# Etienne-bdt/Simple-VAE-RS

Hardware: NVIDIA B200
Metric: train patches/sec (64x64 SR CondVAE, device-timed) (higher is better)
Workload: dtype bf16

## Files before the change

### include/svrs_b200.h

```cpp
#ifndef SVRS_B200_H
#define SVRS_B200_H

#include <stdint.h>

#ifdef __cplusplus
extern "C" {
#endif

#define SVRS_F32 0
#define SVRS_BF16 1

#define SVRS_ACT_NONE 0
#define SVRS_ACT_SIGMOID 1
#define SVRS_ACT_HARDTANH7 2

#define SVRS_E_ARG (-1)
#define SVRS_E_CUDA (-2)
#define SVRS_E_UNSUPPORTED (-3)

const char* svrs_last_error(void);
int svrs_abi_version(void);
int64_t svrs_launch_count(void);
void svrs_trace_reset(int enable);
const char* svrs_trace(void);
int svrs_device_cc(int dev);

int svrs_nchw_to_nhwc(const void* src, int src_dtype, int64_t src_ld, void* dst, int dst_dtype,
                      int N, int C, int H, int W, void* stream);
int svrs_nhwc_to_nchw(const void* src, int src_dtype, void* dst, int dst_dtype, int64_t dst_ld,
                      int N, int C, int H, int W, int accumulate, void* stream);

int svrs_pack_weights(const float* w, int d0, int d1, int kk, void* p01, void* p10, int dtype,
                      void* stream);

int svrs_pack_job_bytes(void);
int svrs_pack_weights_multi(const void* jobs, int njobs, int total_tiles, int max_kk, int dtype, void* stream);
int svrs_unpack_grads_multi(const void* jobs, int njobs, int total_tiles, int max_kk, void* stream);

void svrs_set_tc_enabled(int enabled);
void svrs_set_halo_mode(int mode);
int svrs_tc_would_run(int dtype, int K, int Nc, int OH, int OW);

int svrs_conv2d_fprop(const void* x, const void* w_kn, const void* w_nk, const float* bias, void* y, int dtype,
                      int N, int H, int W, int Cin, int Cout, int ksize, int act, void* stream);
int svrs_conv2d_fprop_ex(const void* x, const void* w_kn, const void* w_nk, const float* bias, void* y, int dtype,
                         int out_dtype, float* y_nchw, int64_t y_nchw_ld, double* bn_sums,
                         int N, int H, int W, int Cin, int Cout, int ksize, int act, void* stream);
int svrs_conv2d_dgrad(const void* dy, const void* w_kn, const void* w_nk, void* dx, int dtype,
                      int N, int H, int W, int Cin, int Cout, int ksize, void* stream);
int svrs_conv2d_wgrad(const void* x, const void* dy, float* dw, float* dw_packed, float* db, int dtype,
                      int N, int H, int W, int Cin, int Cout, int ksize, int ksplit, void* stream);


int svrs_convT2d_fprop(const void* x, const void* w_kn, const void* w_nk, const float* bias, void* y, int dtype,
                       int N, int H, int W, int Cin, int Cout, int act, void* stream);
int svrs_convT2d_fprop_ex(const void* x, const void* w_kn, const void* w_nk, const float* bias, void* y, int dtype,
                          double* bn_sums, int N, int H, int W, int Cin, int Cout, int act, void* stream);
int svrs_convT2d_dgrad(const void* dy, const void* w_kn, const void* w_nk, void* dx, int dtype,
                       int N, int H, int W, int Cin, int Cout, void* stream);
int svrs_convT2d_wgrad(const void* x, const void* dy, float* dw, float* dw_packed, float* db, int dtype,
                       int N, int H, int W, int Cin, int Cout, int ksplit, void* stream);

int svrs_conv2d_wgrad_layout(int dtype, int N, int H, int W, int Cin, int Cout, int ksize);
int svrs_convT2d_wgrad_layout(int dtype, int N, int H, int W, int Cin, int Cout);

#define SVRS_BN_REPLICAS 8
int svrs_bn_stats(const void* x, int dtype, int64_t M, int C, double* sums, void* stream);
int svrs_bn_finalize_train(const double* sums, int64_t M, int C, const float* gamma, const float* beta,
                           float eps, float momentum, float* running_mean, float* running_var,
                           int64_t* num_batches_tracked, int n_updates,
                           float* scale, float* shift, float* mean, float* invstd, void* stream);
int svrs_bn_apply_train(const void* x, void* y, int dtype, int64_t M, int64_t M_stat, int C, const double* sums,
                        const float* gamma, const float* beta, float eps, float momentum,
                        float* running_mean, float* running_var, int64_t* num_batches_tracked, int n_updates,
                        int relu, float* scale, float* shift, float* mean, float* invstd, void* stream);
int svrs_bn_finalize_eval(int C, const float* gamma, const float* beta, float eps,
                          const float* running_mean, const float* running_var,
                          float* scale, float* shift, void* stream);
int svrs_bn_apply(const void* x, void* y, int dtype, int64_t M, int C, const float* scale,
                  const float* shift, int relu, void* stream);
int svrs_bn_bwd_reduce(const void* x, const void* dy, int dtype, int64_t M, int C, const float* scale,
                       const float* shift, const float* mean, const float* invstd, int relu,
                       double* sums, void* stream);
int svrs_bn_bwd_apply(const void* x, const void* dy, void* dx, int dtype, int64_t M, int64_t M_stat, int C,
                      const float* scale, const float* shift, const float* mean, const float* invstd,
                      const float* gamma, int relu, const double* sums, float* dgamma, float* dbeta,
                      void* stream);

int svrs_reparam_fwd(const float* enc, const float* eps, float* z, int64_t z_ld, float* eps_out, int B, int Wd,
                     uint64_t seed, uint32_t stream_id, uint64_t sample_offset, const int64_t* step_ptr,
                     void* stream);
int svrs_reparam_bwd(const float* enc, const float* eps, const float* dz, int64_t dz_ld, float* denc, int B, int Wd,
                     uint64_t seed, uint32_t stream_id, uint64_t sample_offset, const int64_t* step_ptr,
                     void* stream);
int svrs_philox_normal(float* out, int B, int Wd, uint64_t seed, uint32_t stream_id,
                       uint64_t sample_offset, const int64_t* step_ptr, void* stream);

int svrs_elbo_fwd(const void* recon_x, const void* x, int dt_x, int dt_tx, int64_t n_x,
                  const void* recon_y, const void* y, int dt_y, int dt_ty, int64_t n_y,
                  const float* mu1, const float* lv1, int64_t ld1, int W1,
                  const float* mu2, const float* lv2, int64_t ld2,
                  const float* mu3, const float* lv3, int64_t ld3, int W2,
                  int B, double* acc, void* stream);
int svrs_elbo_finalize(const double* acc, int64_t n_x, int64_t n_y, int B, const float* gammas ,
                       float* out5, void* stream);
int svrs_elbo_bwd(const void* recon_x, const void* x, int dt_x, int dt_tx, int64_t n_x, void* d_recon_x, int dt_dx,
                  const void* recon_y, const void* y, int dt_y, int dt_ty, int64_t n_y, void* d_recon_y, int dt_dy,
                  const float* mu1, const float* lv1, int64_t ld1, int W1, float* d_mu1, float* d_lv1, int64_t dld1,
                  const float* mu2, const float* lv2, int64_t ld2, float* d_mu2, float* d_lv2, int64_t dld2,
                  const float* mu3, const float* lv3, int64_t ld3, int W2, float* d_mu3, float* d_lv3, int64_t dld3,
                  int B, const double* acc, const float* gammas, const float* gout, float* d_gammas,
                  int act, void* stream);

int svrs_sumsq(const float* g, int64_t n, double* acc , void* stream);
int svrs_clip_adam(float* p, const float* g, float* m, float* v, int64_t n, const double* sumsq,
                   float max_norm, float grad_scale, float lr, float beta1, float beta2, float eps,
                   const int64_t* step_ptr, void* stream);
int svrs_step_increment(int64_t* step_ptr, void* stream);
int svrs_step_begin(int64_t* step_ptr, double* norm_acc, void* stream);
int svrs_adam_job_bytes(void);
int svrs_adam_tile_rows(void);
int svrs_adam_tile_cols(int kk);
int svrs_adam_multi(const void* jobs, int njobs, int total_tiles, int max_kk, float* p, const float* g, float* m, float* v,
                    int pack_dtype, const double* sumsq, float max_norm, float grad_scale, float lr, float beta1,
                    float beta2, float eps, const int64_t* step_ptr, void* stream);

int svrs_grid_patch_normalize(const void* tiles, int src_is_i16, void* dst, int dst_dtype, int nhwc,
                              int T, int C, int S, int P, void* stream);

int svrs_patch_gather_normalize(const void* tiles, int src_is_i16, int T, int C, int S, int P,
                                const int32_t* origins, int npatch, float* out_nchw_f32, float* out_nhwc_f32,
                                void* out_nhwc_bf16, void* stream);

int svrs_sample_latents(const float* mu3, const float* lv3, int64_t ld3, const float* yflat, int64_t ldy,
                        const float* eps, float* stack, int B, int S, int Wz, uint64_t seed, int stream_id,
                        uint64_t sample_offset, const int64_t* step_ptr, void* stream);
int svrs_sample_tail_splits(int B, int S, int H, int W);
int64_t svrs_sample_tail_scratch_floats(int B, int H, int W, int splits);
int svrs_sample_tail_stats(const void* x, int dtype, const void* w_kn, const float* bias, const float* target_nhwc,
                           int B, int S, int H, int W, int Cin, int Cout, int splits, float* scratch,
                           float* mean_nchw, float* std_map, float* mae_map, float* mse_map, float* bias_map,
                           float* sample0_nchw, void* stream);

int64_t svrs_ssim_workspace_doubles(int N, int C, int H, int W, int win);
int svrs_ssim(const float* a, const float* b, int N, int C, int H, int W, int win, float data_range, double* workspace,
              double* out, void* stream);

int svrs_act_bwd(const void* y, const void* dy, void* dx, int dtype, int act, int64_t n, void* stream);

int svrs_copy2d(const void* src, int src_dtype, int64_t src_ld, void* dst, int dst_dtype, int64_t dst_ld,
                int64_t rows, int cols, int accumulate, void* stream);

int svrs_fill_zero(void* p, int64_t bytes, void* stream);
int svrs_axpy_f32(float* y, const float* x, float a, int64_t n, void* stream);
int svrs_cast(const void* src, int src_dtype, void* dst, int dst_dtype, int64_t n, void* stream);

int svrs_debug_tap_geometry(int form, int N, int H, int W, int Cr, int Cw, int64_t* out, int cap);

#ifdef __cplusplus
}
#endif
#endif
```

### simple-vae-rs_b200/svrs_native/csrc/conv_simt.cu

```cuda
#include "common.cuh"
#include <stdlib.h>
#include "taps.cuh"
#include "tc_ptx.cuh"

namespace svrs {

struct ConvArgs {
    const void* in;
    void* out;
    const void* w;
    const float* bias;
    int act;
    double* bn_sums;
    TapGeom g;
};

constexpr int BK = 16;

}
#include "conv_narrow.cuh"
namespace svrs {
extern int g_tc_enabled_narrow;

template <typename T, int BM, int BN>
// ... 594 lines not shown
#pragma unroll
    for (int j = 0; j < TPW; ++j)
#pragma unroll
        for (int ia = 0; ia < CA; ++ia)
#pragma unroll
            for (int ib = 0; ib < CB; ++ib) {
                float v = acc[j][ia][ib];
#pragma unroll
                for (int o = 16; o > 0; o >>= 1) v += __shfl_xor_sync(0xffffffffu, v, o);
                if (lane == 0) red[warp][(j * CA + ia) * CB + ib] = v;
            }
    __syncwarp();
    for (int e = lane; e < TPW * CA * CB; e += 32) {
        const int ib = e % CB, ia = (e / CB) % CA, j = e / (CA * CB);
        if (t0 + j < pb.ntaps) atomicAdd(&a.dw[((long long)ia * CB + ib) * a.KK + t0 + j], red[warp][e]);
    }
}

template <typename T>
static bool try_launch_wgrad_narrow(const WgradArgs& a, cudaStream_t st, int& rc) {
    const TapGeom& g = a.g;
    const int Ca = g.Nc, Cb = g.K, ntaps = g.prob[0].ntaps;
    const long long ohw = (long long)g.OH * g.OW;
    static const bool disabled = getenv("SVRS_NO_NARROW") != nullptr;
    if (disabled) return false;
    if (g.nprob != 1 || ohw % 32 != 0 || (long long)g.N * ohw >= (1ll << 31) || ntaps > 16) return false;
    const int groups = (int)((long long)g.N * ohw / 32);
    const int warps = (Ca == 4 && Cb == 4) ? (ntaps + 3) / 4 : ntaps;
    const int wpc = warps % 3 == 0 ? 3 : (warps >= 4 ? 4 : warps);
    const int zg = (warps + wpc - 1) / wpc;
    int per_sm = 65536 / (128 * 32 * wpc);
    if (per_sm > 5) per_sm = 5;
    int gx = (num_sms() * per_sm + zg - 1) / zg;
    if (gx > groups) gx = groups;
    dim3 grid(gx, 1, zg);
    if (Ca == 4 && Cb == 16) SVRS_LAUNCH((wgrad_narrow_kernel<T, 4, 16, 1>), grid, 32 * wpc, 0, st, a);
    else if (Ca == 16 && Cb == 4) SVRS_LAUNCH((wgrad_narrow_kernel<T, 16, 4, 1>), grid, 32 * wpc, 0, st, a);
    else if (Ca == 4 && Cb == 4) SVRS_LAUNCH((wgrad_narrow_kernel<T, 4, 4, 4>), grid, 32 * wpc, 0, st, a);
    else return false;
    rc = check_launch("wgrad_narrow_kernel");
    return true;
}

template <typename T>
static int launch_wgrad_direct(const WgradArgs& a, cudaStream_t st) {
    const TapGeom& g = a.g;
    const long long M = (long long)g.N * g.OH * g.OW;
    const int subs = ((g.Nc + 3) / 4) * ((g.K + 3) / 4);
    const int ntaps = g.prob[0].ntaps;
    int SUB = subs <= 1 ? 1 : subs <= 4 ? 4 : subs <= 16 ? 16 : 64;
    int groups = (subs + SUB - 1) / SUB;
    const int L = 256 / SUB;
    long long want = 8LL * num_sms();
    long long split = (want + (long long)ntaps * groups - 1) / ((long long)ntaps * groups);
    long long maxsplit = (M + 8LL * L - 1) / (8LL * L);
    if (split > maxsplit) split = maxsplit;
    if (split < 1) split = 1;
    if (split > 65535) split = 65535;
    dim3 grid(ntaps, (unsigned)split, groups);
    if (SUB == 1) SVRS_LAUNCH((wgrad_direct_kernel<T, 1>), grid, 256, 0, st, a);
    else if (SUB == 4) SVRS_LAUNCH((wgrad_direct_kernel<T, 4>), grid, 256, 0, st, a);
    else if (SUB == 16) SVRS_LAUNCH((wgrad_direct_kernel<T, 16>), grid, 256, 0, st, a);
    else SVRS_LAUNCH((wgrad_direct_kernel<T, 64>), grid, 256, 0, st, a);
    return check_launch("wgrad_direct_kernel");
}

static int launch_wgrad(WgradArgs& a, int dtype, int ksplit, cudaStream_t st) {
    const TapGeom& g = a.g;
    long long M = (long long)g.N * g.OH * g.OW;
    if (M == 0) return 0;
    if ((g.Nc <= 16 || g.K <= 16) && ksplit <= 0) {
        a.ksplit = 1;
        int rc = 0;
        if (dtype == SVRS_F32 ? try_launch_wgrad_narrow<float>(a, st, rc) : try_launch_wgrad_narrow<__nv_bfloat16>(a, st, rc)) return rc;
        return dtype == SVRS_F32 ? launch_wgrad_direct<float>(a, st) : launch_wgrad_direct<__nv_bfloat16>(a, st);
    }
    int tiles = ((g.Nc + 63) / 64) * ((g.K + 63) / 64);
    int ntaps = g.prob[0].ntaps;
    if (ksplit <= 0) {
        long long want = 4LL * num_sms();
        long long base = (long long)tiles * ntaps;
        ksplit = (int)((want + base - 1) / base);
        long long maxsplit = (M + 255) / 256;
        if (ksplit > maxsplit) ksplit = (int)maxsplit;
        if (ksplit < 1) ksplit = 1;
    }
    a.ksplit = ksplit;
    dim3 grid(tiles, ntaps, ksplit);
    if (dtype == SVRS_F32) SVRS_LAUNCH((wgrad_taps_kernel<float>), grid, 256, 0, st, a);
    else SVRS_LAUNCH((wgrad_taps_kernel<__nv_bfloat16>), grid, 256, 0, st, a);
    return check_launch("wgrad_taps_kernel");
}

template <typename T>
__global__ void __launch_bounds__(256) colsum_vec_kernel(const T* __restrict__ x, long long M, int C,
                                                          float* __restrict__ out, long long rows_per_block) {
    pdl_entry();
    __shared__ float red[256][4];
    const int cg = C / 4;
    const int q = threadIdx.x % cg, lane = threadIdx.x / cg, lanes = 256 / cg;
    const long long r0 = (long long)blockIdx.x * rows_per_block;
    long long r1 = r0 + rows_per_block;
    if (r1 > M) r1 = M;
    float4 s = make_float4(0.f, 0.f, 0.f, 0.f);
    for (long long r = r0 + lane; r < r1; r += lanes) {
        float4 v = ld4(x + r * C + q * 4);
        s.x += v.x; s.y += v.y; s.z += v.z; s.w += v.w;
    }
    red[threadIdx.x][0] = s.x; red[threadIdx.x][1] = s.y; red[threadIdx.x][2] = s.z; red[threadIdx.x][3] = s.w;
    __syncthreads();
    if (lane == 0) {
        for (int l = 1; l < lanes; ++l) {
            s.x += red[l * cg + q][0]; s.y += red[l * cg + q][1]; s.z += red[l * cg + q][2]; s.w += red[l * cg + q][3];
        }
        atomicAdd(&out[q * 4 + 0], s.x); atomicAdd(&out[q * 4 + 1], s.y);
        atomicAdd(&out[q * 4 + 2], s.z); atomicAdd(&out[q * 4 + 3], s.w);
    }
}

static int launch_colsum(const void* x, int dtype, long long M, int C, float* out, cudaStream_t st) {
    if (M == 0 || C == 0) return 0;
    if (C % 4 == 0 && C / 4 <= 256 && 256 % (C / 4) == 0) {
        int lanes = 256 / (C / 4);
        long long blocks = (M + (long long)lanes * 16 - 1) / ((long long)lanes * 16);
        long long cap = 4LL * num_sms();
        if (blocks > cap) blocks = cap;
        if (blocks < 1) blocks = 1;
        long long rpb = (M + blocks - 1) / blocks;
        blocks = (M + rpb - 1) / rpb;
        if (dtype == SVRS_F32) SVRS_LAUNCH((colsum_vec_kernel<float>), (unsigned)blocks, 256, 0, st, (const float*)x, M, C, out, rpb);
        else SVRS_LAUNCH((colsum_vec_kernel<__nv_bfloat16>), (unsigned)blocks, 256, 0, st, (const __nv_bfloat16*)x, M, C, out, rpb);
        return check_launch("colsum_vec_kernel");
    }
    long long blocks = (M + 511) / 512;
    long long cap = 8LL * num_sms();
    if (blocks > cap) blocks = cap;
    long long rpb = (M + blocks - 1) / blocks;
    blocks = (M + rpb - 1) / rpb;
    if (dtype == SVRS_F32) SVRS_LAUNCH((colsum_kernel<float>), (unsigned)blocks, 256, 0, st, (const float*)x, M, C, out, rpb);
    else SVRS_LAUNCH((colsum_kernel<__nv_bfloat16>), (unsigned)blocks, 256, 0, st, (const __nv_bfloat16*)x, M, C, out, rpb);
    return check_launch("colsum_kernel");
}

}

namespace svrs {
bool tc_supported(int dtype, int K, int Nc, int OW, int OH);
int launch_conv_tc(int form, const void* in, const void* w_nk, const float* bias, void* out, int N, int H, int W, int Cr, int Cw,
                   int act, const ConvExtra& ex, cudaStream_t st);
bool wgrad_tc_supported(int dtype, int Ca, int Cb, int OW, int OH);
int launch_wgrad_tc(const TapGeom& g, const void* gmat, const void* x, float* dw, int packed, int KK, float* db, cudaStream_t st);
bool wgrad_halo_supported(const TapGeom& g, int KK);
int launch_wgrad3_halo(const TapGeom& g, const void* gmat, const void* x, float* dw, int packed, float* db, cudaStream_t st);
static int g_tc_enabled = 1;
int g_tc_enabled_narrow = 1;
static inline bool use_tc(const void* w_nk, int dtype, int K, int Nc, int OW, int OH) {
    return g_tc_enabled && w_nk != nullptr && !((K == 4 || Nc == 4) && K <= 16 && Nc <= 16) && tc_supported(dtype, K, Nc, OW, OH);
}
}

using namespace svrs;

static bool dtype_ok(int d) { return d == SVRS_F32 || d == SVRS_BF16; }

namespace svrs { void set_halo_mode(int m); }
extern "C" void svrs_set_tc_enabled(int enabled) { svrs::g_tc_enabled = enabled; svrs::g_tc_enabled_narrow = enabled; }
extern "C" void svrs_set_halo_mode(int mode) { svrs::set_halo_mode(mode); }
extern "C" int svrs_tc_would_run(int dtype, int K, int Nc, int OH, int OW) {
    return svrs::g_tc_enabled && svrs::tc_supported(dtype, K, Nc, OW, OH) ? 1 : 0;
}

extern "C" int svrs_conv2d_fprop_ex(const void* x, const void* w_kn, const void* w_nk, const float* bias, void* y, int dtype,
                                    int out_dtype, float* y_nchw, int64_t y_nchw_ld, double* bn_sums,
                                    int N, int H, int W, int Cin, int Cout, int ksize, int act, void* stream) {
    SVRS_CHECK_ARG(x && w_kn && (y || y_nchw) && dtype_ok(dtype) && dtype_ok(out_dtype), "conv2d_fprop: null pointer or bad dtype");
    SVRS_CHECK_ARG(ksize == 3 || (ksize == 4 && H % 2 == 0 && W % 2 == 0), "conv2d_fprop: ksize must be 3, or 4 with even H,W");
    SVRS_CHECK_ARG(N >= 0 && H > 0 && W > 0 && Cin > 0 && Cout > 0, "conv2d_fprop: bad dims");
    if (N > 0 && use_tc(w_nk, dtype, Cin, Cout, ksize == 3 ? W : W / 2, ksize == 3 ? H : H / 2)) {
        if (out_dtype != dtype) { set_error("conv2d_fprop_ex: the tensor-core kernels store bf16 (use y_nchw for an fp32 copy)"); return SVRS_E_UNSUPPORTED; }
        ConvExtra ex;
        ex.out2 = y_nchw; ex.out2_ld = y_nchw_ld; ex.bn_sums = bn_sums;
        return launch_conv_tc(ksize == 3 ? 0 : 2, x, w_nk, bias, y, N, H, W, Cin, Cout, act, ex, (cudaStream_t)stream);
    }
    if (y_nchw || !y) { set_error("conv2d_fprop_ex: the NCHW second output needs the tensor-core kernel (Cin=%d Cout=%d)", Cin, Cout); return SVRS_E_UNSUPPORTED; }
    ConvArgs a;
    a.in = x; a.out = y; a.w = w_kn; a.bias = bias; a.act = act; a.bn_sums = bn_sums;
    if (ksize == 3) geom_conv3(a.g, N, H, W, Cin, Cout, false);
    else geom_conv4s2(a.g, N, H, W, Cin, Cout);
    return launch_conv(a, dtype, (cudaStream_t)stream, out_dtype);
}

extern "C" int svrs_conv2d_fprop(const void* x, const void* w_kn, const void* w_nk, const float* bias, void* y, int dtype,
                                 int N, int H, int W, int Cin, int Cout, int ksize, int act, void* stream) {
    return svrs_conv2d_fprop_ex(x, w_kn, w_nk, bias, y, dtype, dtype, nullptr, 0, nullptr, N, H, W, Cin, Cout, ksize, act, stream);
}

extern "C" int svrs_conv2d_dgrad(const void* dy, const void* w_kn, const void* w_nk, void* dx, int dtype,
                                 int N, int H, int W, int Cin, int Cout, int ksize, void* stream) {
    SVRS_CHECK_ARG(dy && w_kn && dx && dtype_ok(dtype), "conv2d_dgrad: null pointer or bad dtype");
    SVRS_CHECK_ARG(ksize == 3 || (ksize == 4 && H % 2 == 0 && W % 2 == 0), "conv2d_dgrad: ksize must be 3, or 4 with even H,W");
    if (N > 0 && ksize == 3 && use_tc(w_nk, dtype, Cout, Cin, W, H))
        return launch_conv_tc(1, dy, w_nk, nullptr, dx, N, H, W, Cout, Cin, SVRS_ACT_NONE, ConvExtra(), (cudaStream_t)stream);
    if (N > 0 && ksize == 4 && use_tc(w_nk, dtype, Cout, Cin, W / 2, H / 2))
        return launch_conv_tc(3, dy, w_nk, nullptr, dx, N, H / 2, W / 2, Cout, Cin, SVRS_ACT_NONE, ConvExtra(), (cudaStream_t)stream);
    ConvArgs a;
    a.in = dy; a.out = dx; a.w = w_kn; a.bias = nullptr; a.act = SVRS_ACT_NONE; a.bn_sums = nullptr;
    if (ksize == 3) geom_conv3(a.g, N, H, W, Cout, Cin, true);
    else geom_convT4s2(a.g, N, H / 2, W / 2, Cout, Cin);
    return launch_conv(a, dtype, (cudaStream_t)stream);
}

extern "C" int svrs_convT2d_fprop_ex(const void* x, const void* w_kn, const void* w_nk, const float* bias, void* y, int dtype,
                                     double* bn_sums, int N, int H, int W, int Cin, int Cout, int act, void* stream) {
    SVRS_CHECK_ARG(x && w_kn && y && dtype_ok(dtype), "convT2d_fprop: null pointer or bad dtype");
    if (N > 0 && use_tc(w_nk, dtype, Cin, Cout, W, H)) {
        ConvExtra ex;
        ex.bn_sums = bn_sums;
        return launch_conv_tc(3, x, w_nk, bias, y, N, H, W, Cin, Cout, act, ex, (cudaStream_t)stream);
    }
    ConvArgs a;
    a.in = x; a.out = y; a.w = w_kn; a.bias = bias; a.act = act; a.bn_sums = bn_sums;
    geom_convT4s2(a.g, N, H, W, Cin, Cout);
    return launch_conv(a, dtype, (cudaStream_t)stream);
}

extern "C" int svrs_convT2d_fprop(const void* x, const void* w_kn, const void* w_nk, const float* bias, void* y, int dtype,
                                  int N, int H, int W, int Cin, int Cout, int act, void* stream) {
    return svrs_convT2d_fprop_ex(x, w_kn, w_nk, bias, y, dtype, nullptr, N, H, W, Cin, Cout, act, stream);
}

extern "C" int svrs_convT2d_dgrad(const void* dy, const void* w_kn, const void* w_nk, void* dx, int dtype,
                                  int N, int H, int W, int Cin, int Cout, void* stream) {
    SVRS_CHECK_ARG(dy && w_kn && dx && dtype_ok(dtype), "convT2d_dgrad: null pointer or bad dtype");
    if (N > 0 && use_tc(w_nk, dtype, Cout, Cin, W, H))
        return launch_conv_tc(2, dy, w_nk, nullptr, dx, N, 2 * H, 2 * W, Cout, Cin, SVRS_ACT_NONE, ConvExtra(), (cudaStream_t)stream);
    ConvArgs a;
    a.in = dy; a.out = dx; a.w = w_kn; a.bias = nullptr; a.act = SVRS_ACT_NONE; a.bn_sums = nullptr;
    geom_conv4s2(a.g, N, 2 * H, 2 * W, Cout, Cin);
    return launch_conv(a, dtype, (cudaStream_t)stream);
}

extern "C" int svrs_conv2d_wgrad(const void* x, const void* dy, float* dw, float* dw_packed, float* db, int dtype,
                                 int N, int H, int W, int Cin, int Cout, int ksize, int ksplit, void* stream) {
    SVRS_CHECK_ARG(x && dy && dtype_ok(dtype), "conv2d_wgrad: null pointer or bad dtype");
    SVRS_CHECK_ARG(ksize == 3 || (ksize == 4 && H % 2 == 0 && W % 2 == 0), "conv2d_wgrad: bad ksize");
    int rc = 0;
    if (dw) {
        WgradArgs a;
        a.gmat = dy; a.x = x; a.dw = dw; a.KK = ksize * ksize;
        if (ksize == 3) geom_conv3(a.g, N, H, W, Cin, Cout, false);
        else geom_conv4s2(a.g, N, H, W, Cin, Cout);
        const bool fold_db = db != nullptr && Cout % 8 == 0;
        if (g_tc_enabled_narrow && ksplit <= 0 && wgrad16_takes(dtype, N, H, W, Cin, Cout, ksize)) {
            rc = launch_wgrad16(x, dy, dw, db, N, H, W, Cin, (cudaStream_t)stream);
            db = nullptr;
        } else if (g_tc_enabled && N > 0 && dtype == SVRS_BF16 && wgrad_halo_supported(a.g, a.KK)) {
            rc = launch_wgrad3_halo(a.g, dy, x, dw_packed ? dw_packed : dw, dw_packed != nullptr, fold_db ? db : nullptr, (cudaStream_t)stream);
            if (fold_db) db = nullptr;
        } else if (g_tc_enabled && N > 0 && wgrad_tc_supported(dtype, Cout, Cin, a.g.OW, a.g.OH)) {
            rc = launch_wgrad_tc(a.g, dy, x, dw_packed ? dw_packed : dw, dw_packed != nullptr, a.KK, fold_db ? db : nullptr, (cudaStream_t)stream);
            if (fold_db) db = nullptr;
        } else if (g_tc_enabled_narrow && N > 0 && ksplit <= 0 && wgrad_narrow_mma_takes(a.g, dtype)) {
            rc = launch_wgrad_narrow_mma(a, db, (cudaStream_t)stream);
            db = nullptr;
        } else
            rc = launch_wgrad(a, dtype, ksplit, (cudaStream_t)stream);
        if (rc) return rc;
    }
    if (db) {
        int s = ksize == 3 ? 1 : 2;
        rc = launch_colsum(dy, dtype, (long long)N * (H / s) * (W / s), Cout, db, (cudaStream_t)stream);
    }
    return rc;
}

extern "C" int svrs_convT2d_wgrad(const void* x, const void* dy, float* dw, float* dw_packed, float* db, int dtype,
                                  int N, int H, int W, int Cin, int Cout, int ksplit, void* stream) {
    SVRS_CHECK_ARG(x && dy && dtype_ok(dtype), "convT2d_wgrad: null pointer or bad dtype");
    int rc = 0;
    if (dw) {
        WgradArgs a;
        a.gmat = x; a.x = dy; a.dw = dw; a.KK = 16;
        geom_conv4s2(a.g, N, 2 * H, 2 * W, Cout, Cin);
        if (g_tc_enabled && N > 0 && wgrad_tc_supported(dtype, Cin, Cout, a.g.OW, a.g.OH))
            rc = launch_wgrad_tc(a.g, x, dy, dw_packed ? dw_packed : dw, dw_packed != nullptr, 16, nullptr, (cudaStream_t)stream);
        else
            rc = launch_wgrad(a, dtype, ksplit, (cudaStream_t)stream);
        if (rc) return rc;
    }
    if (db) rc = launch_colsum(dy, dtype, (long long)N * 4 * H * W, Cout, db, (cudaStream_t)stream);
    return rc;
}

extern "C" int svrs_conv2d_wgrad_layout(int dtype, int N, int H, int W, int Cin, int Cout, int ksize) {
    if (!(ksize == 3 || (ksize == 4 && H % 2 == 0 && W % 2 == 0)) || N <= 0) return 0;
    if (g_tc_enabled_narrow && wgrad16_takes(dtype, N, H, W, Cin, Cout, ksize)) return 0;
    TapGeom g;
    if (ksize == 3) geom_conv3(g, N, H, W, Cin, Cout, false);
    else geom_conv4s2(g, N, H, W, Cin, Cout);
    if (g_tc_enabled && dtype == SVRS_BF16 && wgrad_halo_supported(g, ksize * ksize)) return 1;
    if (g_tc_enabled && wgrad_tc_supported(dtype, Cout, Cin, g.OW, g.OH)) return 1;
    return 0;
}
extern "C" int svrs_convT2d_wgrad_layout(int dtype, int N, int H, int W, int Cin, int Cout) {
    if (N <= 0) return 0;
    TapGeom g;
    geom_conv4s2(g, N, 2 * H, 2 * W, Cout, Cin);
    return (g_tc_enabled && wgrad_tc_supported(dtype, Cin, Cout, g.OW, g.OH)) ? 1 : 0;
}

extern "C" int svrs_debug_tap_geometry(int form, int N, int H, int W, int Cr, int Cw, int64_t* out, int cap) {
    SVRS_CHECK_ARG(out && form >= 0 && form <= 3, "debug_tap_geometry: bad args");
    TapGeom g;
    if (form == 0) geom_conv3(g, N, H, W, Cr, Cw, false);
    else if (form == 1) geom_conv3(g, N, H, W, Cr, Cw, true);
    else if (form == 2) geom_conv4s2(g, N, H, W, Cr, Cw);
    else geom_convT4s2(g, N, H, W, Cr, Cw);
    int n = 0;
    auto put = [&](long long v) { if (n < cap) out[n] = v; ++n; };
    put(g.N); put(g.OH); put(g.OW); put(g.IH); put(g.IW); put(g.K); put(g.Nc); put(g.nprob);
    put(g.o_sn); put(g.o_sy); put(g.o_sx); put(g.i_sn); put(g.i_sy); put(g.i_sx);
    for (int p = 0; p < g.nprob; ++p) {
        put(g.prob[p].out_off); put(g.prob[p].ntaps);
        for (int t = 0; t < g.prob[p].ntaps; ++t) {
            put(g.prob[p].taps[t].in_off); put(g.prob[p].taps[t].w_off); put(g.prob[p].taps[t].dy); put(g.prob[p].taps[t].dx);
        }
    }
    SVRS_CHECK_ARG(n <= cap, "debug_tap_geometry: buffer too small (%d needed)", n);
    return n;
}
```

### simple-vae-rs_b200/svrs_native/lib.py

```python
from __future__ import annotations

import ctypes
import os
import re
from typing import Dict, List, Tuple

HERE = os.path.dirname(os.path.abspath(__file__))
ROOT = os.path.dirname(os.path.dirname(HERE))
HEADER = os.path.join(ROOT, "include", "svrs_b200.h")
LIB_PATH = os.path.join(HERE, "libsvrs_b200.so")

F32, BF16 = 0, 1
ACT_NONE, ACT_SIGMOID, ACT_HARDTANH7 = 0, 1, 2

_SCALARS = {
    "int": ctypes.c_int,
    "int64_t": ctypes.c_int64,
    "uint64_t": ctypes.c_uint64,
    "uint32_t": ctypes.c_uint32,
    "float": ctypes.c_float,
}


class SvrsError(RuntimeError):
    pass


class SvrsUnsupported(SvrsError):
    """SVRS_E_UNSUPPORTED (-3): the kernel that takes this shape cannot provide a requested optional extra; nothing was
    enqueued.  Callers use the separate kernels instead (never a CPU path)."""


def parse_header(path: str = HEADER) -> Dict[str, Tuple[str, List[Tuple[str, str]]]]:
    src = open(path).read()
    src = re.sub(r"/\*.*?\*/", " ", src, flags=re.S)
    src = re.sub(r"//[^\n]*", " ", src)
    protos = {}
    for m in re.finditer(r"(const\s+char\s*\*|int64_t|int|void)\s+(svrs_\w+)\s*\(([^;{]*?)\)\s*;", src, flags=re.S):
        ret, name, args = m.group(1), m.group(2), m.group(3)
        arglist = []
        args = " ".join(args.split())
        if args and args != "void":
            for a in args.split(","):
                a = a.strip()
                mm = re.match(r"(.*?)(\w+)$", a)
                ty, an = mm.group(1).strip(), mm.group(2)
                arglist.append((ty.replace(" *", "*"), an))
        protos[name] = ("char*" if "char" in ret else ret.strip(), arglist)
    return protos


def _ctype(ty: str):
    if "*" in ty:
        return ctypes.c_void_p
    ty = ty.replace("const", "").strip()
    return _SCALARS[ty]


class _Lib:
    def __init__(self):
        self._dll = None
        self.protos = parse_header()
        self.timing = None
        self.timing_pad_cycles = 0

    def load(self):
        if self._dll is not None:
            return self._dll
        if not os.path.exists(LIB_PATH):
            raise SvrsError(
                f"{LIB_PATH} is missing: the sm_100a kernel library has not been built "
                f"(run `python simple-vae-rs_b200/svrs_native/build.py`). There is no CPU/eager fallback.")
        dll = ctypes.CDLL(LIB_PATH)
        for name, (ret, args) in self.protos.items():
            fn = getattr(dll, name)
            fn.argtypes = [_ctype(t) for t, _ in args]
            fn.restype = {"char*": ctypes.c_char_p, "void": None, "int64_t": ctypes.c_int64}.get(ret, ctypes.c_int)
        self._dll = dll
        return dll

    def last_error(self) -> str:
        return self.load().svrs_last_error().decode()

    def __getattr__(self, name):
        full = "svrs_" + name
        if full not in self.protos:
            raise AttributeError(name)
        fn = getattr(self.load(), full)
        if self.protos[full][0] != "int" or full in ("svrs_abi_version", "svrs_device_cc", "svrs_debug_tap_geometry", "svrs_tc_would_run", "svrs_pack_job_bytes", "svrs_launch_count", "svrs_adam_job_bytes", "svrs_adam_tile_rows", "svrs_adam_tile_cols",
                                                  "svrs_conv2d_wgrad_layout", "svrs_convT2d_wgrad_layout", "svrs_sample_tail_splits"):
            setattr(self, name, fn)
            return fn

        def call(*a, _fn=fn, _n=full):
            if self.timing is not None:
                import torch
                e0, e1 = torch.cuda.Event(enable_timing=True), torch.cuda.Event(enable_timing=True)
                if self.timing_pad_cycles:
                    torch.cuda._sleep(self.timing_pad_cycles)
                dll = self.load()
                dll.svrs_trace_reset(1)
                e0.record()
                rc = _fn(*a)
                e1.record()
                kernels = dll.svrs_trace().decode()
                dll.svrs_trace_reset(0)
                self.timing.append((_n, a, e0, e1, kernels))
            else:
                rc = _fn(*a)
            if rc == -3:
                raise SvrsUnsupported(f"{_n}: {self.last_error()}")
            if rc != 0:
                raise SvrsError(f"{_n} failed ({rc}): {self.last_error()}")

        setattr(self, name, call)
        return call


lib = _Lib()


def require_cuda_library():
    lib.load()
    return LIB_PATH
```

Measured before the change: 46780.

## Add halo-tiled tcgen05 wgrad kernel for 4x4 stride-2 conv and convT

```diff
diff --git a/include/svrs_b200.h b/include/svrs_b200.h
--- a/include/svrs_b200.h
+++ b/include/svrs_b200.h
@@ -63,6 +63,14 @@
 
 int svrs_conv2d_wgrad_layout(int dtype, int N, int H, int W, int Cin, int Cout, int ksize);
 int svrs_convT2d_wgrad_layout(int dtype, int N, int H, int W, int Cin, int Cout);
+
+#define SVRS_WG_SIMT 0
+#define SVRS_WG_NARROW_MMA 1
+#define SVRS_WG_16 2
+#define SVRS_WG_TC 3
+#define SVRS_WG_3_HALO 4
+#define SVRS_WG_4S2_HALO 5
+int svrs_wgrad_kernel(int transposed, int dtype, int N, int H, int W, int Cin, int Cout, int ksize);
 
 #define SVRS_BN_REPLICAS 8
 int svrs_bn_stats(const void* x, int dtype, int64_t M, int C, double* sums, void* stream);
diff --git a/simple-vae-rs_b200/svrs_native/csrc/conv_simt.cu b/simple-vae-rs_b200/svrs_native/csrc/conv_simt.cu
--- a/simple-vae-rs_b200/svrs_native/csrc/conv_simt.cu
+++ b/simple-vae-rs_b200/svrs_native/csrc/conv_simt.cu
@@ -770,6 +770,8 @@
 int launch_wgrad_tc(const TapGeom& g, const void* gmat, const void* x, float* dw, int packed, int KK, float* db, cudaStream_t st);
 bool wgrad_halo_supported(const TapGeom& g, int KK);
 int launch_wgrad3_halo(const TapGeom& g, const void* gmat, const void* x, float* dw, int packed, float* db, cudaStream_t st);
+bool wgrad4s2_halo_supported(const TapGeom& g, int KK);
+int launch_wgrad4s2_halo(const TapGeom& g, const void* gmat, const void* x, float* dw, int packed, float* db, int db_fine, cudaStream_t st);
 static int g_tc_enabled = 1;
 int g_tc_enabled_narrow = 1;
 static inline bool use_tc(const void* w_nk, int dtype, int K, int Nc, int OW, int OH) {
@@ -858,6 +860,27 @@
     return launch_conv(a, dtype, (cudaStream_t)stream);
 }
 
+static int wgrad_choice(int convT, int dtype, int N, int H, int W, int Cin, int Cout, int ksize, int ksplit, WgradArgs& a) {
+    if (convT) {
+        a.KK = 16;
+        geom_conv4s2(a.g, N, 2 * H, 2 * W, Cout, Cin);
+        if (g_tc_enabled && N > 0 && dtype == SVRS_BF16 && wgrad4s2_halo_supported(a.g, 16)) return SVRS_WG_4S2_HALO;
+        if (g_tc_enabled && N > 0 && wgrad_tc_supported(dtype, Cin, Cout, a.g.OW, a.g.OH)) return SVRS_WG_TC;
+        return SVRS_WG_SIMT;
+    }
+    a.KK = ksize * ksize;
+    if (ksize == 3) geom_conv3(a.g, N, H, W, Cin, Cout, false);
+    else geom_conv4s2(a.g, N, H, W, Cin, Cout);
+    if (g_tc_enabled_narrow && ksplit <= 0 && wgrad16_takes(dtype, N, H, W, Cin, Cout, ksize)) return SVRS_WG_16;
+    if (g_tc_enabled && N > 0 && dtype == SVRS_BF16 && wgrad_halo_supported(a.g, a.KK)) return SVRS_WG_3_HALO;
+    if (g_tc_enabled && N > 0 && dtype == SVRS_BF16 && wgrad4s2_halo_supported(a.g, a.KK)) return SVRS_WG_4S2_HALO;
+    if (g_tc_enabled && N > 0 && wgrad_tc_supported(dtype, Cout, Cin, a.g.OW, a.g.OH)) return SVRS_WG_TC;
+    if (g_tc_enabled_narrow && N > 0 && ksplit <= 0 && wgrad_narrow_mma_takes(a.g, dtype)) return SVRS_WG_NARROW_MMA;
+    return SVRS_WG_SIMT;
+}
+
+static bool wgrad_packed(int kernel) { return kernel == SVRS_WG_TC || kernel == SVRS_WG_3_HALO || kernel == SVRS_WG_4S2_HALO; }
+
 extern "C" int svrs_conv2d_wgrad(const void* x, const void* dy, float* dw, float* dw_packed, float* db, int dtype,
                                  int N, int H, int W, int Cin, int Cout, int ksize, int ksplit, void* stream) {
     SVRS_CHECK_ARG(x && dy && dtype_ok(dtype), "conv2d_wgrad: null pointer or bad dtype");
@@ -865,24 +888,36 @@
     int rc = 0;
     if (dw) {
         WgradArgs a;
-        a.gmat = dy; a.x = x; a.dw = dw; a.KK = ksize * ksize;
-        if (ksize == 3) geom_conv3(a.g, N, H, W, Cin, Cout, false);
-        else geom_conv4s2(a.g, N, H, W, Cin, Cout);
+        a.gmat = dy; a.x = x; a.dw = dw;
+        const int kernel = wgrad_choice(0, dtype, N, H, W, Cin, Cout, ksize, ksplit, a);
+        float* dwk = wgrad_packed(kernel) && dw_packed ? dw_packed : dw;
+        const int packed = wgrad_packed(kernel) && dw_packed != nullptr;
         const bool fold_db = db != nullptr && Cout % 8 == 0;
-        if (g_tc_enabled_narrow && ksplit <= 0 && wgrad16_takes(dtype, N, H, W, Cin, Cout, ksize)) {
-            rc = launch_wgrad16(x, dy, dw, db, N, H, W, Cin, (cudaStream_t)stream);
+        cudaStream_t st = (cudaStream_t)stream;
+        switch (kernel) {
+        case SVRS_WG_16:
+            rc = launch_wgrad16(x, dy, dw, db, N, H, W, Cin, st);
             db = nullptr;
-        } else if (g_tc_enabled && N > 0 && dtype == SVRS_BF16 && wgrad_halo_supported(a.g, a.KK)) {
-            rc = launch_wgrad3_halo(a.g, dy, x, dw_packed ? dw_packed : dw, dw_packed != nullptr, fold_db ? db : nullptr, (cudaStream_t)stream);
+            break;
+        case SVRS_WG_3_HALO:
+            rc = launch_wgrad3_halo(a.g, dy, x, dwk, packed, fold_db ? db : nullptr, st);
             if (fold_db) db = nullptr;
-        } else if (g_tc_enabled && N > 0 && wgrad_tc_supported(dtype, Cout, Cin, a.g.OW, a.g.OH)) {
-            rc = launch_wgrad_tc(a.g, dy, x, dw_packed ? dw_packed : dw, dw_packed != nullptr, a.KK, fold_db ? db : nullptr, (cudaStream_t)stream);
+            break;
+        case SVRS_WG_4S2_HALO:
+            rc = launch_wgrad4s2_halo(a.g, dy, x, dwk, packed, fold_db ? db : nullptr, 0, st);
             if (fold_db) db = nullptr;
-        } else if (g_tc_enabled_narrow && N > 0 && ksplit <= 0 && wgrad_narrow_mma_takes(a.g, dtype)) {
-            rc = launch_wgrad_narrow_mma(a, db, (cudaStream_t)stream);
+            break;
+        case SVRS_WG_TC:
+            rc = launch_wgrad_tc(a.g, dy, x, dwk, packed, a.KK, fold_db ? db : nullptr, st);
+            if (fold_db) db = nullptr;
+            break;
+        case SVRS_WG_NARROW_MMA:
+            rc = launch_wgrad_narrow_mma(a, db, st);
             db = nullptr;
-        } else
-            rc = launch_wgrad(a, dtype, ksplit, (cudaStream_t)stream);
+            break;
+        default:
+            rc = launch_wgrad(a, dtype, ksplit, st);
+        }
         if (rc) return rc;
     }
     if (db) {
@@ -898,10 +933,15 @@
     int rc = 0;
     if (dw) {
         WgradArgs a;
-        a.gmat = x; a.x = dy; a.dw = dw; a.KK = 16;
-        geom_conv4s2(a.g, N, 2 * H, 2 * W, Cout, Cin);
-        if (g_tc_enabled && N > 0 && wgrad_tc_supported(dtype, Cin, Cout, a.g.OW, a.g.OH))
-            rc = launch_wgrad_tc(a.g, x, dy, dw_packed ? dw_packed : dw, dw_packed != nullptr, 16, nullptr, (cudaStream_t)stream);
+        a.gmat = x; a.x = dy; a.dw = dw;
+        const int kernel = wgrad_choice(1, dtype, N, H, W, Cin, Cout, 4, ksplit, a);
+        float* dwk = wgrad_packed(kernel) && dw_packed ? dw_packed : dw;
+        const int packed = wgrad_packed(kernel) && dw_packed != nullptr;
+        if (kernel == SVRS_WG_4S2_HALO) {
+            rc = launch_wgrad4s2_halo(a.g, x, dy, dwk, packed, db, 1, (cudaStream_t)stream);
+            db = nullptr;
+        } else if (kernel == SVRS_WG_TC)
+            rc = launch_wgrad_tc(a.g, x, dy, dwk, packed, 16, nullptr, (cudaStream_t)stream);
         else
             rc = launch_wgrad(a, dtype, ksplit, (cudaStream_t)stream);
         if (rc) return rc;
@@ -910,21 +950,22 @@
     return rc;
 }
 
+extern "C" int svrs_wgrad_kernel(int transposed, int dtype, int N, int H, int W, int Cin, int Cout, int ksize) {
+    SVRS_CHECK_ARG(dtype_ok(dtype) && (transposed ? ksize == 4 : (ksize == 3 || (ksize == 4 && H % 2 == 0 && W % 2 == 0))),
+                   "wgrad_kernel: bad dtype or ksize");
+    WgradArgs a;
+    return wgrad_choice(transposed, dtype, N, H, W, Cin, Cout, ksize, 0, a);
+}
+
 extern "C" int svrs_conv2d_wgrad_layout(int dtype, int N, int H, int W, int Cin, int Cout, int ksize) {
     if (!(ksize == 3 || (ksize == 4 && H % 2 == 0 && W % 2 == 0)) || N <= 0) return 0;
-    if (g_tc_enabled_narrow && wgrad16_takes(dtype, N, H, W, Cin, Cout, ksize)) return 0;
-    TapGeom g;
-    if (ksize == 3) geom_conv3(g, N, H, W, Cin, Cout, false);
-    else geom_conv4s2(g, N, H, W, Cin, Cout);
-    if (g_tc_enabled && dtype == SVRS_BF16 && wgrad_halo_supported(g, ksize * ksize)) return 1;
-    if (g_tc_enabled && wgrad_tc_supported(dtype, Cout, Cin, g.OW, g.OH)) return 1;
-    return 0;
+    WgradArgs a;
+    return wgrad_packed(wgrad_choice(0, dtype, N, H, W, Cin, Cout, ksize, 0, a)) ? 1 : 0;
 }
 extern "C" int svrs_convT2d_wgrad_layout(int dtype, int N, int H, int W, int Cin, int Cout) {
     if (N <= 0) return 0;
-    TapGeom g;
-    geom_conv4s2(g, N, 2 * H, 2 * W, Cout, Cin);
-    return (g_tc_enabled && wgrad_tc_supported(dtype, Cin, Cout, g.OW, g.OH)) ? 1 : 0;
+    WgradArgs a;
+    return wgrad_packed(wgrad_choice(1, dtype, N, H, W, Cin, Cout, 4, 0, a)) ? 1 : 0;
 }
 
 extern "C" int svrs_debug_tap_geometry(int form, int N, int H, int W, int Cr, int Cw, int64_t* out, int cap) {
diff --git a/simple-vae-rs_b200/svrs_native/csrc/wgrad4s2_halo.cu b/simple-vae-rs_b200/svrs_native/csrc/wgrad4s2_halo.cu
--- /dev/null
+++ b/simple-vae-rs_b200/svrs_native/csrc/wgrad4s2_halo.cu
@@ -0,0 +1,290 @@
+#include "common.cuh"
+#include "taps.cuh"
+#include "tc_ptx.cuh"
+#include <string.h>
+#include <stdlib.h>
+
+namespace svrs {
+
+constexpr int W4_PITCH = 9;
+constexpr int W4_G_BYTES = 128 * 128 * 2;
+constexpr int W4_THREADS = 192;
+constexpr int W4_MAX_STAGES = 3;
+constexpr int W4_SMEM_EXTRA = 1024 + 256;
+constexpr int W4_SMEM_LIMIT = W4_MAX_STAGES * (2 * 20480 + W4_G_BYTES) + W4_SMEM_EXTRA;
+
+__device__ __forceinline__ uint4 ld_shared_v4(uint32_t addr) {
+    uint4 r;
+    asm volatile("ld.shared.v4.b32 {%0, %1, %2, %3}, [%4];" : "=r"(r.x), "=r"(r.y), "=r"(r.z), "=r"(r.w) : "r"(addr) : "memory");
+    return r;
+}
+
+struct alignas(64) W4Params {
+    CUtensorMap x_maps[4];
+    CUtensorMap g_map;
+    CUtensorMap dw_map;
+    float* dw;
+    float* db;
+    const __nv_bfloat16* gptr;
+    long long g_sn, g_sy, g_sx;
+    int N, BH, BNI, tiles_x, tiles_y;
+    int Ca, Cb, a_tiles, b_chunks, ksplit, ksteps_total, packed, db_fine;
+    int halo_bytes, halo_slot, stage_bytes, stages;
+};
+
+__global__ void __launch_bounds__(W4_THREADS, 1) wgrad4s2_halo_kernel(const __grid_constant__ W4Params p) {
+    pdl_entry();
+    extern __shared__ uint8_t smem_raw[];
+    const uint32_t smem_base = (smem_u32(smem_raw) + 1023u) & ~1023u;
+    const uint32_t bar_base = smem_base + (uint32_t)(p.stages * p.stage_bytes);
+    auto full_bar = [&](int s) { return bar_base + 8u * s; };
+    auto empty_bar = [&](int s) { return bar_base + 8u * (W4_MAX_STAGES + s); };
+    const uint32_t done_bar = bar_base + 8u * (2 * W4_MAX_STAGES);
+    const uint32_t tmem_slot = bar_base + 8u * (2 * W4_MAX_STAGES + 1);
+    uint32_t* tmem_slot_ptr = reinterpret_cast<uint32_t*>(smem_raw + (tmem_slot - smem_u32(smem_raw)));
+    const int warp = threadIdx.x / 32, lane = threadIdx.x % 32;
+    int w = blockIdx.x;
+    const int py = w % 2; w /= 2;
+    const int bj = w % p.b_chunks; w /= p.b_chunks;
+    const int at = w % p.a_tiles; w /= p.a_tiles;
+    const int ks = w;
+    const int steps_per = (p.ksteps_total + p.ksplit - 1) / p.ksplit;
+    const int k_begin = ks * steps_per;
+    const int k_end = (k_begin + steps_per) < p.ksteps_total ? (k_begin + steps_per) : p.ksteps_total;
+    const int nsteps = k_end > k_begin ? k_end - k_begin : 0;
+    const bool halo_db = p.db != nullptr && p.db_fine && at == 0;
+
+    if (warp == 0 && lane == 0) {
+        for (int i = 0; i < 4; ++i) prefetch_tmap(&p.x_maps[i]);
+        prefetch_tmap(&p.g_map);
+        if (p.packed) prefetch_tmap(&p.dw_map);
+        for (int s = 0; s < p.stages; ++s) { mbar_init(full_bar(s), 1); mbar_init(empty_bar(s), halo_db ? 5 : 1); }
+        mbar_init(done_bar, 1);
+        asm volatile("fence.mbarrier_init.release.cluster;" ::: "memory");
+    }
+    if (warp == 1) {
+        asm volatile("tcgen05.alloc.cta_group::1.sync.aligned.shared::cta.b32 [%0], 512;" ::"r"(tmem_slot) : "memory");
+        asm volatile("tcgen05.relinquish_alloc_permit.cta_group::1.sync.aligned;" ::: "memory");
+    }
+    tc_fence_before();
+    __syncthreads();
+    tc_fence_after();
+    const uint32_t tmem_base = *tmem_slot_ptr;
+    pdl_wait();
+
+
+    if (warp == 0) {
+        if (lane == 0) {
+            int stage = 0;
+            uint32_t phase = 0;
+            for (int kstep = k_begin; kstep < k_end; ++kstep) {
+                int pt = kstep;
+                const int tx = pt % p.tiles_x; pt /= p.tiles_x;
+                const int ty = pt % p.tiles_y;
+                const int n0 = (pt / p.tiles_y) * p.BNI;
+                const int x0 = tx * 8, y0 = ty * p.BH;
+                mbar_wait(empty_bar(stage), phase ^ 1u);
+                const uint32_t sh = smem_base + (uint32_t)(stage * p.stage_bytes);
+                mbar_expect_tx(full_bar(stage), (uint32_t)(2 * p.halo_bytes + W4_G_BYTES));
+                for (int px = 0; px < 2; ++px)
+                    tma_load_4d(sh + (uint32_t)(px * p.halo_slot), &p.x_maps[py * 2 + px], full_bar(stage), bj * 64, x0 - px, y0 - py, n0);
+                const uint32_t sg = sh + (uint32_t)(2 * p.halo_slot);
+                for (int c = 0; c < 2; ++c)
+                    tma_load_4d(sg + (uint32_t)c * 16384u, &p.g_map, full_bar(stage), at * 128 + c * 64, x0, y0, n0);
+                if (++stage == p.stages) { stage = 0; phase ^= 1u; }
+            }
+        }
+    } else if (warp == 1) {
+        if (lane == 0) {
+            const uint32_t idesc = (1u << 4) | (1u << 7) | (1u << 10) | (1u << 15) | (1u << 16) | ((128u >> 3) << 17) | ((128u >> 4) << 24);
+            const uint32_t a_hi = desc_hi(W4_PITCH * 128u, 2u), b_hi = desc_hi(1024u, 2u);
+            const uint32_t a_lbo = (128u >> 4) << 16;
+            uint32_t koff[8];
+#pragma unroll
+            for (int k = 0; k < 8; ++k) koff[k] = (uint32_t)(((2 * k) / p.BH * (p.BH + 1) + (2 * k) % p.BH) * W4_PITCH * 8);
+            int stage = 0;
+            uint32_t phase = 0;
+            for (int kstep = 0; kstep < nsteps; ++kstep) {
+                mbar_wait(full_bar(stage), phase);
+                tc_fence_after();
+                const uint32_t sh = smem_base + (uint32_t)(stage * p.stage_bytes);
+                const uint32_t a0 = ((sh & 0x3FFFF) >> 4) | a_lbo;
+                const uint32_t b0 = desc_lo(sh + (uint32_t)(2 * p.halo_slot), 16384u);
+                const uint32_t hs = (uint32_t)p.halo_slot >> 4;
+#pragma unroll
+                for (int k = 0; k < 8; ++k)
+#pragma unroll
+                    for (int pr = 0; pr < 4; ++pr)
+                        tc_mma_lohi(tmem_base + (uint32_t)(pr * 128), a0 + (pr >> 1) * hs + (pr & 1) * (W4_PITCH * 8) + koff[k], a_hi,
+                                    b0 + 128u * k, b_hi, idesc, k ? 1u : (uint32_t)(kstep != 0));
+                tc_commit(empty_bar(stage));
+                if (kstep == nsteps - 1) tc_commit(done_bar);
+                if (++stage == p.stages) { stage = 0; phase ^= 1u; }
+            }
+        }
+    } else if (nsteps > 0) {
+        const int q = warp % 4;
+        const int m = q * 32 + lane;
+        __shared__ float csum[128][8];
+        const int t = threadIdx.x - 64;
+        float acc[8] = {0.f, 0.f, 0.f, 0.f, 0.f, 0.f, 0.f, 0.f};
+        if (halo_db) {
+            const int cq = t % 8, cl = t / 8;
+            int stage = 0;
+            uint32_t phase = 0;
+            for (int kstep = 0; kstep < nsteps; ++kstep) {
+                mbar_wait(full_bar(stage), phase);
+                const uint32_t sh = smem_base + (uint32_t)(stage * p.stage_bytes);
+#pragma unroll
+                for (int px = 0; px < 2; ++px)
+#pragma unroll
+                    for (int j = 0; j < 8; ++j) {
+                        const int pix = cl + 16 * j, img = pix / (8 * p.BH), iy = (pix / 8) % p.BH, ix = pix % 8;
+                        const uint32_t row = (uint32_t)(((img * (p.BH + 1) + iy + py) * W4_PITCH) + ix + px);
+                        const uint4 r = ld_shared_v4(sh + (uint32_t)(px * p.halo_slot) + row * 128u + ((cq ^ (row & 7u)) << 4));
+                        const uint32_t wv[4] = {r.x, r.y, r.z, r.w};
+#pragma unroll
+                        for (int e = 0; e < 4; ++e) { acc[2 * e] += __uint_as_float(wv[e] << 16); acc[2 * e + 1] += __uint_as_float(wv[e] & 0xffff0000u); }
+                    }
+                __syncwarp();
+                if (lane == 0) mbar_arrive(empty_bar(stage));
+                if (++stage == p.stages) { stage = 0; phase ^= 1u; }
+            }
+            colsum_finish(csum, acc, t, cq, cl, 8, 16, p.db, bj * 64, p.Cb);
+        } else if (p.db && !p.db_fine) {
+            const int r = py + 2 * bj, nr = 2 * p.b_chunks;
+            const int cq = t % 16, cl = t / 16;
+            for (int kstep = k_begin + r; kstep < k_end; kstep += nr) {
+                int pt = kstep;
+                const int tx = pt % p.tiles_x; pt /= p.tiles_x;
+                const int ty = pt % p.tiles_y;
+                const int n0 = (pt / p.tiles_y) * p.BNI;
+                colsum_tile8(p.gptr, p.g_sn, p.g_sy, p.g_sx, n0, ty * p.BH, 8 * tx, 8, p.BH, p.BNI, p.N, at * 128 + cq * 8, cl, 8, acc);
+            }
+            colsum_finish(csum, acc, t, cq, cl, 16, 8, p.db, at * 128, p.Ca);
+        }
+        mbar_wait(done_bar, 0);
+        tc_fence_after();
+        const int h = m >> 6, r = m & 63;
+        auto tap_of = [&](int pr, int hh) { return (2 * (pr & 1) + 1 - py) * 4 + 2 * hh + 1 - (pr >> 1); };
+        if (p.packed) {
+            const bool issuer = threadIdx.x == 64;
+            for (int u = 0; u < 8; ++u) {
+                const int pr = u >> 1, c64 = (u & 1) * 64;
+                const uint32_t buf = smem_base + (uint32_t)(u & 1) * 32768u;
+                if (u >= 2) {
+                    if (issuer) bulk_wait_read_1();
+                    named_bar_sync(1, 128);
+                }
+                const uint32_t taddr = tmem_base + (uint32_t)(pr * 128 + c64) + ((uint32_t)(q * 32) << 16);
+#pragma unroll
+                for (int c0 = 0; c0 < 64; c0 += 32) {
+                    uint32_t v[32];
+                    tmem_ld32(taddr + c0, v);
+                    tmem_ld_wait();
+                    stage_row_swizzled<8>(buf + (uint32_t)(h * 2 + c0 / 32) * 8192u, r, 128u, v);
+                }
+                fence_proxy_async_smem();
+                named_bar_sync(1, 128);
+                if (issuer) {
+                    for (int hh = 0; hh < 2; ++hh)
+                        for (int cc = 0; cc < 2; ++cc)
+                            tma_reduce_add_2d(&p.dw_map, buf + (uint32_t)(hh * 2 + cc) * 8192u, at * 128 + c64 + cc * 32,
+                                              tap_of(pr, hh) * p.Cb + bj * 64);
+                    bulk_commit();
+                }
+            }
+            if (issuer) bulk_wait_all();
+        } else {
+            const int cb = bj * 64 + r;
+            for (int pr = 0; pr < 4; ++pr) {
+                const int tap = tap_of(pr, h);
+                const uint32_t taddr = tmem_base + (uint32_t)(pr * 128) + ((uint32_t)(q * 32) << 16);
+                for (int c0 = 0; c0 < 128; c0 += 32) {
+                    uint32_t v[32];
+                    tmem_ld32(taddr + c0, v);
+                    tmem_ld_wait();
+#pragma unroll
+                    for (int j = 0; j < 32; ++j) {
+                        const int ca = at * 128 + c0 + j;
+                        atomicAdd(p.dw + ((long long)ca * p.Cb + cb) * 16 + tap, __uint_as_float(v[j]));
+                    }
+                }
+            }
+        }
+    }
+
+    tc_fence_before();
+    __syncthreads();
+    if (warp == 1) {
+        tc_fence_after();
+        asm volatile("tcgen05.dealloc.cta_group::1.sync.aligned.b32 %0, 512;" ::"r"(tmem_base) : "memory");
+    }
+}
+
+int get_halo_mode();
+
+bool wgrad4s2_halo_supported(const TapGeom& g, int KK) {
+    static const bool env_on = [] { const char* e = getenv("SVRS_WG4_HALO"); return !(e && atoi(e) == 0); }();
+    return env_on && get_halo_mode() != 0 && KK == 16 && g.nprob == 1 && g.prob[0].ntaps == 16 && g.Nc % 128 == 0 &&
+           g.K % 64 == 0 && g.OW % 8 == 0 && g.OH % 8 == 0 && g.IH == g.OH && g.IW == g.OW;
+}
+
+static void w4_plan(const TapGeom& g, W4Params& p) {
+    memset(&p, 0, sizeof(p));
+    p.N = g.N;
+    p.BH = g.OH % 16 == 0 ? 16 : 8;
+    p.BNI = 128 / (8 * p.BH);
+    p.tiles_x = g.OW / 8; p.tiles_y = g.OH / p.BH;
+    p.Ca = g.Nc; p.Cb = g.K;
+    p.a_tiles = p.Ca / 128; p.b_chunks = p.Cb / 64;
+    p.ksteps_total = p.tiles_x * p.tiles_y * ((g.N + p.BNI - 1) / p.BNI);
+    p.halo_bytes = 128 * W4_PITCH * (p.BH + 1) * p.BNI;
+    p.halo_slot = (p.halo_bytes + 1023) & ~1023;
+    p.stage_bytes = 2 * p.halo_slot + W4_G_BYTES;
+    p.stages = (W4_SMEM_LIMIT - W4_SMEM_EXTRA) / p.stage_bytes;
+    if (p.stages > W4_MAX_STAGES) p.stages = W4_MAX_STAGES;
+    const int base = p.a_tiles * p.b_chunks * 2;
+    static const int target = getenv("SVRS_WG4_CTAS") ? atoi(getenv("SVRS_WG4_CTAS"))
+                            : getenv("SVRS_WG_TARGET_CTAS") ? atoi(getenv("SVRS_WG_TARGET_CTAS")) : num_sms() / 2;
+    int ksplit = (target + base / 2) / base;
+    if (ksplit > p.ksteps_total / 4) ksplit = p.ksteps_total / 4;
+    if (ksplit < 1) ksplit = 1;
+    const int steps_per = (p.ksteps_total + ksplit - 1) / ksplit;
+    p.ksplit = (p.ksteps_total + steps_per - 1) / steps_per;
+}
+
+int launch_wgrad4s2_halo(const TapGeom& g, const void* gmat, const void* x, float* dw, int packed, float* db, int db_fine, cudaStream_t st) {
+    static bool attr_set = false;
+    if (!attr_set) {
+        cudaError_t e = cudaFuncSetAttribute(wgrad4s2_halo_kernel, cudaFuncAttributeMaxDynamicSharedMemorySize, W4_SMEM_LIMIT);
+        if (e != cudaSuccess) { set_error("wgrad4s2_halo: cudaFuncSetAttribute: %s", cudaGetErrorString(e)); return SVRS_E_CUDA; }
+        attr_set = true;
+    }
+    W4Params p;
+    w4_plan(g, p);
+    p.dw = dw;
+    p.packed = packed;
+    p.db = db;
+    p.db_fine = db_fine;
+    p.gptr = reinterpret_cast<const __nv_bfloat16*>(gmat);
+    p.g_sn = g.o_sn; p.g_sy = g.o_sy; p.g_sx = g.o_sx;
+    const Prob& pb = g.prob[0];
+    const __nv_bfloat16* xb = reinterpret_cast<const __nv_bfloat16*>(x);
+    for (int par = 0; par < 4; ++par) {
+        const long long off = pb.taps[(1 - par / 2) * 4 + 1 - par % 2].in_off;
+        int rc = make_act_map(&p.x_maps[par], xb + off, p.Cb, g.IW, g.IH, g.N, g.i_sx, g.i_sy, g.i_sn, W4_PITCH, p.BH + 1, p.BNI, 64);
+        if (rc) return rc;
+    }
+    int rc = make_act_map(&p.g_map, gmat, p.Ca, g.OW, g.OH, g.N, g.o_sx, g.o_sy, g.o_sn, 8, p.BH, p.BNI, 64);
+    if (rc) return rc;
+    if (packed) {
+        rc = make_f32_2d_map(&p.dw_map, dw, p.Ca, 16ll * p.Cb, 32, 64);
+        if (rc) return rc;
+    }
+    const int grid = p.a_tiles * p.b_chunks * 2 * p.ksplit;
+    SVRS_LAUNCH((wgrad4s2_halo_kernel), grid, W4_THREADS, p.stages * p.stage_bytes + W4_SMEM_EXTRA, st, p);
+    return check_launch("wgrad4s2_halo_kernel");
+}
+
+}
diff --git a/simple-vae-rs_b200/svrs_native/lib.py b/simple-vae-rs_b200/svrs_native/lib.py
--- a/simple-vae-rs_b200/svrs_native/lib.py
+++ b/simple-vae-rs_b200/svrs_native/lib.py
@@ -88,7 +88,7 @@
             raise AttributeError(name)
         fn = getattr(self.load(), full)
         if self.protos[full][0] != "int" or full in ("svrs_abi_version", "svrs_device_cc", "svrs_debug_tap_geometry", "svrs_tc_would_run", "svrs_pack_job_bytes", "svrs_launch_count", "svrs_adam_job_bytes", "svrs_adam_tile_rows", "svrs_adam_tile_cols",
-                                                  "svrs_conv2d_wgrad_layout", "svrs_convT2d_wgrad_layout", "svrs_sample_tail_splits"):
+                                                  "svrs_conv2d_wgrad_layout", "svrs_convT2d_wgrad_layout", "svrs_wgrad_kernel", "svrs_sample_tail_splits"):
             setattr(self, name, fn)
             return fn
 
```

After: 46720, median of 6. No clear change (-0.1%).
